# jasperzhong/GNNFlow

Measured on AMD Instinct MI355X. Metric: sampled_edges_per_s, higher is better.
Workload: dtype int64/f32

## Files before the change

### gnnflow_amd/csrc/cache_lru.hip

```cpp
#include "cache_lru_dev.hpp"

#include <algorithm>

namespace gf {

namespace {


__global__ __launch_bounds__(kWide, 8) void lru_list_scan_kernel(Round r, uint32_t row_blocks,
                                                              uint32_t list_blocks,
                                                              uint32_t victim_blocks) {
  const Ctx& c = r.c[blockIdx.y];
  if (!c.update || c.policy != GF_CACHE_LRU || c.fused) return;
  const int tid = threadIdx.x;
  __shared__ uint32_t ws[kWide / 64];
  const uint32_t parity = c.qstate->parity;
  const uint32_t* list = c.queue[parity & 1u];
  constexpr uint32_t kItems = kRowTile / kWide;
  if (blockIdx.x < row_blocks) {
    __shared__ uint32_t carry;
    const uint32_t row_tiles = (c.n + kLruRows - 1) / kLruRows;
    constexpr uint32_t kItems = kLruRows / kWide;
    const uint32_t t_begin = blockIdx.x * c.tiles_per_wg;
    if (t_begin >= row_tiles) return;
    const uint32_t t_end = min(t_begin + c.tiles_per_wg, row_tiles);
    if (tid == 0) carry = 0;
    __syncthreads();
    for (uint32_t t = t_begin; t < t_end; ++t) {
      const uint32_t i0 = t * kLruRows + tid * kItems;
      int32_t sr[kItems];
      int64_t idv[kItems];
#pragma unroll
      for (uint32_t k = 0; k < kItems; ++k) {
        const bool ok = i0 + k < c.n;
        sr[k] = ok ? c.slot_of_row[i0 + k] : -2;
        idv[k] = ok ? c.ids[i0 + k] : 0;
      }
      if (t == t_begin && total_miss(c.ctr) == 0) return;
      uint32_t fm[kItems], lm = 0;
#pragma unroll
      for (uint32_t k = 0; k < kItems; ++k) {
        fm[k] = (sr[k] == -1 && c.map[idv[k]] == -static_cast<int32_t>(i0 + k + 1)) ? 1u : 0u;
        lm += fm[k];
      }
      uint32_t tm;
      uint32_t run = carry + wide_excl_scan(lm, ws, &tm);
#pragma unroll
      for (uint32_t k = 0; k < kItems; ++k) {
        if (i0 + k < c.n && (fm[k] || !c.qmode)) c.rep_flag[i0 + k] = fm[k] ? (kRepMiss | run) : 0u;
        run += fm[k];
      }
      __syncthreads();
      if (tid == 0) carry += tm;
      __syncthreads();
    }
    if (tid == 0) c.row_tile_sum[blockIdx.x] = carry;
    return;
  }
  const uint32_t cap = c.capacity;
  if (blockIdx.x < row_blocks + list_blocks) {
    if (c.qmode) {
      const uint32_t head = c.qstate->head, tail = c.qstate->tail;
      const uint32_t w_lo = head >> 5, w_hi = (tail + 31u) >> 5;
      const uint32_t t0 = w_lo / kBitTile;
      const uint32_t btiles = (w_hi + kBitTile - 1) / kBitTile - t0;
      const bool none = total_miss(c.ctr) == 0;
      for (uint32_t t = blockIdx.x - row_blocks; t < btiles; t += list_blocks) {
        const size_t wi = static_cast<size_t>(t0 + t) * kBitTile + tid * 4;
        const uint4 wd = *reinterpret_cast<const uint4*>(c.qbits + wi);
        if (none) {
          if (wd.x | wd.y | wd.z | wd.w) *reinterpret_cast<uint4*>(c.qbits + wi) = make_uint4(0u, 0u, 0u, 0u);
          continue;
        }
        const uint32_t p0 = __popc(wd.x), p1 = __popc(wd.y), p2 = __popc(wd.z), p3 = __popc(wd.w);
        uint32_t total;
        const uint32_t b = wide_excl_scan(p0 + p1 + p2 + p3, ws, &total);
        uint4* sn = reinterpret_cast<uint4*>(c.wsnap + wi);
        if (wd.x | wd.y) sn[0] = make_uint4(wd.x, b, wd.y, b + p0);
        if (wd.z | wd.w) sn[1] = make_uint4(wd.z, b + p0 + p1, wd.w, b + p0 + p1 + p2);
        if (tid == 0) c.tile_tie[t] = total;
      }
      return;
    }
    const uint32_t list_tiles = (cap + kRowTile - 1) / kRowTile;
    if (blockIdx.x == row_blocks && tid == 0) c.ctr->q_parity = parity;
    bool first = true, staged = false;
    for (uint32_t t = blockIdx.x - row_blocks; t < list_tiles; t += list_blocks) {
      const uint32_t p0 = t * kRowTile + tid * kItems;
      uint32_t sl[kItems], hit[kItems], tc[kItems], local = 0;
#pragma unroll
      for (uint32_t j = 0; j < kItems; ++j) tc[j] = p0 + j < cap ? c.touched[p0 + j] : 0u;
      if (first) {
        uint32_t alt[kItems];
#pragma unroll
        for (uint32_t j = 0; j < kItems; ++j) {
          sl[j] = p0 + j < cap ? c.queue[0][p0 + j] : 0u;
          alt[j] = p0 + j < cap ? c.queue[1][p0 + j] : 0u;
        }
#pragma unroll
        for (uint32_t j = 0; j < kItems; ++j) sl[j] = (parity & 1u) ? alt[j] : sl[j];
        first = false;
        const uint32_t missed = total_miss(c.ctr);
        if (missed == 0) return;
        staged = use_staged_victims(c.stage_tiles, missed, c.stage_min);
      } else {
#pragma unroll
        for (uint32_t j = 0; j < kItems; ++j) sl[j] = p0 + j < cap ? list[p0 + j] : 0u;
      }
#pragma unroll
      for (uint32_t j = 0; j < kItems; ++j) {
        hit[j] = (p0 + j < cap && tc[j] == c.epoch_new) ? 1u : 0u;
        local += hit[j];
      }
      uint32_t total;
      if (staged && t < c.stage_tiles) {
        uint32_t before_hits = wide_excl_scan(local, ws, &total);
        uint32_t at_keep = t * kRowTile + tid * kItems - before_hits;
        uint32_t at_hit = t * kRowTile + before_hits;
#pragma unroll
        for (uint32_t j = 0; j < kItems; ++j) {
          if (p0 + j < cap) {
            if (!hit[j]) c.v_slot[at_keep++] = sl[j];
            else if (c.stage_hits) c.v_pos[at_hit++] = sl[j];
          }
        }
      } else {
        total = wide_sum(local, ws);
      }
      if (tid == 0) {
        c.tile_tie[t] = total;
        if (total) atomicAdd(&c.tile_old[t / kQGroup], total);
      }
    }
    return;
  }
  const uint32_t want = min(total_miss(c.ctr), cap);
  if (c.qmode) {
    const uint32_t vb = blockIdx.x - row_blocks - list_blocks;
    const uint32_t head = c.qstate->head, tail = c.qstate->tail;
    if (vb == 0 && tid == 0) { c.ctr->q_parity = parity; c.ctr->q_head = head; c.ctr->q_tail = tail; }
    if (want == 0) return;
    const uint32_t hbase = head & ~3u, chunks = victim_chunks_used(c, want);
    for (uint32_t ch = vb; ch < chunks; ch += victim_blocks) {
      const uint32_t p0 = hbase + ch * kRowTile + tid * 4;
      uint32_t sl[4];
      const uint32_t mask = victim_walk4(c, list, head, tail, p0, sl);
      uint32_t total;
      uint32_t at = ch * kRowTile + wide_excl_scan(__popc(mask), ws, &total);
#pragma unroll
      for (uint32_t j = 0; j < 4; ++j)
        if (mask & (1u << j)) { c.v_slot[at] = sl[j]; c.v_pos[at] = p0 + j; ++at; }
      if (tid == 0) c.v_count[ch] = total;
    }
    return;
  }
  if (blockIdx.x != row_blocks + list_blocks ||
      use_staged_victims(c.stage_tiles, total_miss(c.ctr), c.stage_min)) return;
  if (want == 0) return;
  uint32_t* kept = c.rep_row;
  uint32_t* moved = c.rep_rank;
  uint32_t found = 0, found_hit = 0;
  for (uint32_t base = 0; base < cap && found < want; base += kRowTile) {
    const uint32_t p0 = base + tid * kItems;
    uint32_t sl[kItems], hit[kItems], lk = 0, lh = 0;
#pragma unroll
    for (uint32_t j = 0; j < kItems; ++j) sl[j] = p0 + j < cap ? list[p0 + j] : 0u;
#pragma unroll
    for (uint32_t j = 0; j < kItems; ++j) {
      const bool in = p0 + j < cap;
      hit[j] = in ? (c.touched[p0 + j] == c.epoch_new ? 1u : 0u) : 2u;
      lk += hit[j] == 0u;
      lh += hit[j] == 1u;
    }
    uint32_t tk, th;
    uint32_t ik = found + wide_excl_scan(lk, ws, &tk);
    uint32_t ih = found_hit + wide_excl_scan(lh, ws, &th);
#pragma unroll
    for (uint32_t j = 0; j < kItems; ++j) {
      if (hit[j] == 0u) { if (ik < want) kept[ik] = sl[j]; ++ik; }
      else if (hit[j] == 1u) { if (ih < want) moved[ih] = sl[j]; ++ih; }
    }
    found += tk;
    found_hit += th;
  }
  if (tid == 0) c.ctr->q_found = min(found, want);
}

__global__ __launch_bounds__(kWide) void lru_list_install_kernel(Round r, uint32_t row_blocks,
                                                                 uint32_t list_blocks) {
  const Ctx& c = r.c[blockIdx.y];
  if (!c.update || c.policy != GF_CACHE_LRU || c.fused || c.qmode) return;
  const int tid = threadIdx.x;
  __shared__ uint32_t ws[kWide / 64];
  const uint32_t row_tiles = (c.n + kLruRows - 1) / kLruRows;
  const uint32_t spans = (row_tiles + c.tiles_per_wg - 1) / c.tiles_per_wg;
  const uint32_t cap = c.capacity;
  if (blockIdx.x < row_blocks) {
    __shared__ uint2 inst[kWide];
    __shared__ int64_t inst_id[kWide];
    __shared__ uint32_t n_inst;
    __shared__ uint32_t s_keep[kMaxStageTiles], s_hitp[kMaxStageTiles], s_nonhit;
    const uint32_t span_rows = c.tiles_per_wg * kLruRows;
    const uint32_t inst_rows = c.inst_rows;
    const uint32_t chunks = (c.n + inst_rows - 1) / inst_rows;
    for (uint32_t chunk = blockIdx.x; chunk < chunks; chunk += row_blocks) {
      const uint32_t i = chunk * inst_rows + tid;
      const bool in = tid < static_cast<int>(inst_rows) && i < c.n;
      const uint32_t code = in ? c.rep_flag[i] : 0u;
      const int64_t id = in ? c.ids[i] : 0;
      const uint32_t w = (chunk * inst_rows) / span_rows;
      uint32_t pm = 0, tm = 0;
      for (uint32_t t = tid; t < spans; t += kWide) {
        const uint32_t m = c.row_tile_sum[t];
        tm += m;
        if (t < w) pm += m;
      }
      const uint32_t q_found = c.ctr->q_found;
      const bool staged = use_staged_victims(c.stage_tiles, total_miss(c.ctr), c.stage_min);
      uint32_t stage_hit = 0, stage_len = 0, th_part = 0;
      if (staged && chunk == blockIdx.x) {
        if (tid < static_cast<int>(c.stage_tiles)) {
          stage_hit = c.tile_tie[tid];
          stage_len = min(kRowTile, cap - tid * kRowTile);
        }
        const uint32_t groups = ((cap + kRowTile - 1) / kRowTile + kQGroup - 1) / kQGroup;
        for (uint32_t g = tid; g < groups; g += kWide) th_part += c.tile_old[g];
      }
      if (chunk == blockIdx.x && total_miss(c.ctr) == 0) return;
      pm = wide_sum(pm, ws);
      tm = wide_sum(tm, ws);
      if (staged && chunk == blockIdx.x) {
        uint32_t unused;
        const uint32_t th = wide_sum(th_part, ws);
        const uint32_t keep_before = wide_excl_scan(stage_len - stage_hit, ws, &unused);
        const uint32_t hit_before = wide_excl_scan(stage_hit, ws, &unused);
        if (tid < static_cast<int>(kMaxStageTiles)) {
          s_keep[tid] = keep_before;
          s_hitp[tid] = hit_before;
        }
        if (tid == 0) s_nonhit = cap - th;
      }
      if (tid == 0) n_inst = 0;
      __syncthreads();
      const uint32_t k = min(tm, cap);
      if (code & kRepMiss) {
        const uint32_t m = pm + (code & kRepRank);
        if (m < k) {
          uint32_t slot;
          int64_t old;
          if (staged) {
            const bool keep = m < s_nonhit;
            const uint32_t x = keep ? m : m - s_nonhit;
            const uint32_t* pref = keep ? s_keep : s_hitp;
            uint32_t lo = 0, hi = c.stage_tiles;
            while (hi - lo > 1) {
              const uint32_t mid = (lo + hi) >> 1;
              if (pref[mid] <= x) lo = mid; else hi = mid;
            }
            const uint32_t at = lo * kRowTile + (x - pref[lo]);
            slot = (keep ? c.v_slot : c.v_pos)[at];
            old = c.slot_id[slot];
          } else {
            slot = m < q_found ? c.rep_row[m] : c.rep_rank[m - q_found];
            old = c.slot_id[slot];
          }
          if (old >= 0) c.map[old] = kAbsent;
          c.slot_id[slot] = id;
          c.map[id] = static_cast<int32_t>(slot);
          const uint32_t at = atomicAdd(&n_inst, 1u);
          inst[at] = make_uint2(slot, i);
          inst_id[at] = id;
        } else {
          c.map[id] = kAbsent;
        }
      }
      __syncthreads();
      const uint32_t total = n_inst * c.dimv;
      if (c.vec4) {
        if (c.inst_rows > kInstRows) copy_installed<float4, 6>(c, inst, inst_id, n_inst, c.dimv * 4, tid);
        else copy_installed<float4, 2>(c, inst, inst_id, n_inst, c.dimv * 4, tid);
      } else if (c.odd4) {
        if (c.inst_rows > kInstRows) copy_installed<uf4, 6>(c, inst, inst_id, n_inst, c.dim, tid);
        else copy_installed<uf4, 2>(c, inst, inst_id, n_inst, c.dim, tid);
      } else {
        for (uint32_t f = tid; c.cache_buf && f < total; f += kWide) {
          const uint32_t j = f / c.dimv, cc = f - j * c.dimv;
          const uint2 pr = inst[j];
          c.cache_buf[static_cast<uint64_t>(pr.x) * c.dimv + cc] =
              c.inst_from_table ? c.feats[static_cast<uint64_t>(inst_id[j]) * c.dimv + cc]
                                : c.out[static_cast<uint64_t>(pr.y) * c.dimv + cc];
        }
      }
      __syncthreads();
    }
    return;
  }
  if (blockIdx.x >= row_blocks + list_blocks) return;
  const uint32_t parity = c.ctr->q_parity;
  const uint32_t* list = c.queue[parity & 1u];
  uint32_t* next = c.queue[(parity & 1u) ^ 1u];
  constexpr uint32_t kSubs = kRowTile / kWide;
  const uint32_t list_tiles = (cap + kRowTile - 1) / kRowTile;
  const uint32_t sub_tiles = (cap + kWide - 1) / kWide;
  const uint32_t groups = (list_tiles + kQGroup - 1) / kQGroup;
  const uint32_t st_first = blockIdx.x - row_blocks;
  uint32_t sl0, tc0;
  {
    const uint32_t p = st_first * kWide + tid;
    const uint32_t a0 = p < cap ? c.queue[0][p] : 0u;
    const uint32_t a1 = p < cap ? c.queue[1][p] : 0u;
    tc0 = p < cap ? c.touched[p] : 0u;
    sl0 = (parity & 1u) ? a1 : a0;
  }
  uint32_t tm = 0, th = 0;
  for (uint32_t t = tid; t < spans; t += kWide) tm += c.row_tile_sum[t];
  for (uint32_t g = tid; g < groups; g += kWide) th += c.tile_old[g];
  if (total_miss(c.ctr) == 0) return;
  tm = wide_sum(tm, ws);
  th = wide_sum(th, ws);
  const uint32_t k = min(tm, cap), n_kept = cap - th;
  for (uint32_t st = st_first; st < sub_tiles; st += list_blocks) {
    const uint32_t t = st / kSubs, q = st - t * kSubs;
    const uint32_t p = st * kWide + tid;
    uint32_t sl, tc;
    if (st == st_first) {
      sl = sl0; tc = tc0;
    } else {
      sl = p < cap ? list[p] : 0u;
      tc = p < cap ? c.touched[p] : 0u;
    }
    uint32_t before = 0;
    const uint32_t g0 = t / kQGroup;
    for (uint32_t g = tid; g < g0; g += kWide) before += c.tile_old[g];
    for (uint32_t u = g0 * kQGroup + tid; u < t; u += kWide) before += c.tile_tie[u];
    for (uint32_t j = 0; j < q; ++j) {
      const uint32_t pj = t * kRowTile + j * kWide + tid;
      before += (pj < cap && c.touched[pj] == c.epoch_new) ? 1u : 0u;
    }
    const uint32_t hit = (p < cap && tc == c.epoch_new) ? 1u : 0u;
    before = wide_sum(before, ws);
    uint32_t total;
    const uint32_t hb = before + wide_excl_scan(hit, ws, &total);
    if (p < cap) {
      const uint32_t l = hit ? n_kept + hb : p - hb;
      const uint32_t at = l < k ? cap - k + l : l - k;
      next[at] = sl;
      c.qpos[sl] = at;
    }
  }
  if (blockIdx.x == row_blocks && tid == 0) c.qstate->parity = parity ^ 1u;
}

__global__ void list_fill_kernel(uint32_t* list, uint32_t first, uint32_t prefix,
                                 const uint32_t* old, uint32_t old_n) {
  const uint32_t stride = gridDim.x * blockDim.x;
  for (uint32_t j = blockIdx.x * blockDim.x + threadIdx.x; j < prefix + old_n; j += stride)
    list[j] = j < prefix ? first + j : old[j - prefix];
}
void lru_list_fill(uint32_t* list, uint32_t first, uint32_t prefix, const uint32_t* old,
                   uint32_t old_n, hipStream_t stream) {
  list_fill_kernel<<<dim3(1024), dim3(256), 0, stream>>>(list, first, prefix, old, old_n);
  GF_HIP(hipGetLastError());
}

struct RoundFork {
  hipStream_t side = nullptr;
  hipEvent_t begin = nullptr, end = nullptr;
  int device = -1;
  ~RoundFork() {
    if (side) (void)hipStreamDestroy(side);
    if (begin) (void)hipEventDestroy(begin);
    if (end) (void)hipEventDestroy(end);
  }
};
inline RoundFork& round_fork() {
  static thread_local RoundFork f;
  return f;
}
inline bool fork_round(hipStream_t stream, hipStream_t* side) {
  RoundFork& f = round_fork();
  int dev = 0;
  GF_HIP(hipGetDevice(&dev));
  if (f.side && f.device != dev) return false;
  if (!f.side) {
    GF_HIP(hipStreamCreateWithFlags(&f.side, hipStreamNonBlocking));
    GF_HIP(hipEventCreateWithFlags(&f.begin, hipEventDisableTiming));
    GF_HIP(hipEventCreateWithFlags(&f.end, hipEventDisableTiming));
    f.device = dev;
  }
  GF_HIP(hipEventRecord(f.begin, stream));
  GF_HIP(hipStreamWaitEvent(f.side, f.begin, 0));
  *side = f.side;
  return true;
}
inline void fork_done() { GF_HIP(hipEventRecord(round_fork().end, round_fork().side)); }
inline void join_round(hipStream_t stream) { GF_HIP(hipStreamWaitEvent(stream, round_fork().end, 0)); }

struct LruExtents {
  size_t fused_list_tiles = 0;
  size_t fused_row_wgs = 0;
  size_t scan_rows = 0;
  size_t scan_row_wgs = 0;
  size_t list_capacity = 0;
  size_t list_inst_wgs = 0;
  size_t queue_bit_tiles = 0;
  size_t queue_victim_wgs = 1;
  size_t queue_rows = 0;
};

LruExtents lru_extents(const Round& r) {
  LruExtents x;
  for (int i = 0; i < r.count; ++i) {
    const Ctx& c = r.c[i];
    if (!c.update || c.policy != GF_CACHE_LRU) continue;
    if (c.fused) {
      x.fused_list_tiles = std::max<size_t>(x.fused_list_tiles, (c.capacity + kFuseTile - 1) / kFuseTile);
      x.fused_row_wgs = std::max<size_t>(x.fused_row_wgs, (c.n + c.fuse_rows - 1) / c.fuse_rows);
      continue;
    }
    const size_t row_tiles = (c.n + kLruRows - 1) / kLruRows;
    x.scan_rows = std::max<size_t>(x.scan_rows, c.n);
    x.scan_row_wgs = std::max(x.scan_row_wgs, (row_tiles + c.tiles_per_wg - 1) / c.tiles_per_wg);
    if (c.qmode) {
      x.queue_bit_tiles = std::max(x.queue_bit_tiles, lru_bit_tiles(c.capacity));
      x.queue_victim_wgs = std::max<size_t>(x.queue_victim_wgs, std::min<size_t>(c.v_chunks, 1024));
      x.queue_rows = std::max<size_t>(x.queue_rows, c.n);
    } else {
      x.list_capacity = std::max<size_t>(x.list_capacity, c.capacity);
      x.list_inst_wgs = std::max<size_t>(x.list_inst_wgs, (c.n + c.inst_rows - 1) / c.inst_rows);
    }
  }
  return x;
}

void launch_list_scan(const Round& r, const LruExtents& x, hipStream_t stream) {
  const unsigned rb = static_cast<unsigned>(x.scan_row_wgs);
  const unsigned lb = static_cast<unsigned>(std::min<size_t>(
      std::max((x.list_capacity + kRowTile - 1) / kRowTile, x.queue_bit_tiles), 1024));
  const unsigned vb = static_cast<unsigned>(x.queue_victim_wgs);
  lru_list_scan_kernel<<<dim3(rb + lb + vb, r.count), dim3(kWide), 0, stream>>>(r, rb, lb, vb);
}

void launch_list_install(const Round& r, const LruExtents& x, hipStream_t stream) {
  const unsigned ib = static_cast<unsigned>(std::min<size_t>(x.list_inst_wgs, 4096));
  const unsigned lb = std::max<unsigned>(
      1, static_cast<unsigned>(std::min<size_t>((x.list_capacity + kWide - 1) / kWide, 1024)));
  lru_list_install_kernel<<<dim3(ib + lb, r.count), dim3(kWide), 0, stream>>>(r, ib, lb);
}

}

void launch_lru_update(const Round& r, hipStream_t stream, bool own_events) {
  const LruExtents x = lru_extents(r);
  hipStream_t side = nullptr;
  const bool forked = x.fused_list_tiles && x.scan_rows && fork_round(stream, &side);
  if (x.fused_list_tiles) {
    launch_lru_fused(r, x.fused_list_tiles, x.fused_row_wgs, forked ? side : stream, own_events);
    if (forked) fork_done();
  }
  if (x.scan_rows) {
    launch_list_scan(r, x, stream);
    if (x.queue_bit_tiles) launch_lru_queue_update(r, x.queue_rows, stream);
    if (x.list_inst_wgs) launch_list_install(r, x, stream);
    GF_HIP(hipGetLastError());
    if (forked) join_round(stream);
  }
}

void FeatureCache::alloc_queue(size_t capacity, hipStream_t stream, DeviceBuffer* old_lists) {
  const bool queue_form = capacity >= queue_min_capacity();
  const size_t queue_cap = lru_queue_cap(capacity, queue_form);
  GF_REQUIRE(!queue_form || queue_cap < (size_t{1} << 30),
             "LRU queue form: more than 2^30 queue positions");
  queue_form_ = queue_form;
  queue_cap_ = queue_cap;
  if (old_lists) {
    old_lists[0] = std::move(queue_);
    old_lists[1] = std::move(queue_alt_);
  }
  auto place = [&](DeviceBuffer& buf, size_t bytes) {
    if (!old_lists) {
      buf.reserve(bytes, 0, stream);
    } else {
      DeviceBuffer fresh;
      fresh.reserve(bytes);
      std::swap(buf, fresh);
    }
  };
  const size_t list_bytes = (queue_cap_ + 16) * sizeof(uint32_t);
  place(queue_, list_bytes);
  place(queue_alt_, list_bytes);
  place(qpos_, std::max<size_t>(capacity, 4) * sizeof(uint32_t));
  if (queue_form_) {
    place(wsnap_, 2 * qbits_bytes(queue_cap_));
    place(qbits_, qbits_bytes(queue_cap_));
    GF_HIP(hipMemsetAsync(qbits_.data(), 0, qbits_bytes(queue_cap_), stream));
    place(compact_, compact_layout(queue_cap_).bytes);
  } else if (!old_lists) {
    wsnap_.release();
    qbits_.release();
    compact_.release();
  }
}

void FeatureCache::init_queue(hipStream_t stream) {
  if (policy_ != GF_CACHE_LRU) return;
  alloc_queue(capacity_, stream, nullptr);
  if (capacity_) lru_list_fill(queue_.as<uint32_t>(), 0u, static_cast<uint32_t>(capacity_), nullptr, 0u, stream);
  const QueueState qs{0u, 0u, 0u, static_cast<uint32_t>(capacity_), 0u, 0u};
  GF_HIP(hipMemcpyAsync(qstate_.data(), &qs, sizeof(qs), hipMemcpyHostToDevice, stream));
  GF_HIP(hipStreamSynchronize(stream));
  tail_bound_ = capacity_;
  index_queue(stream);
}

void FeatureCache::grow_queue(size_t old_capacity, hipStream_t stream) {
  QueueState qs;
  GF_HIP(hipMemcpyAsync(&qs, qstate_.data(), sizeof(qs), hipMemcpyDeviceToHost, stream));
  GF_HIP(hipStreamSynchronize(stream));
  DeviceBuffer old_lists[2];
  alloc_queue(capacity_, stream, old_lists);
  lru_list_fill(queue_.as<uint32_t>(), static_cast<uint32_t>(old_capacity),
                static_cast<uint32_t>(capacity_ - old_capacity), old_lists[qs.parity & 1u].as<uint32_t>(),
                static_cast<uint32_t>(old_capacity), stream);
  const QueueState fresh{0u, 0u, 0u, static_cast<uint32_t>(capacity_), 0u, 0u};
  GF_HIP(hipMemcpyAsync(qstate_.data(), &fresh, sizeof(fresh), hipMemcpyHostToDevice, stream));
  GF_HIP(hipStreamSynchronize(stream));
  tail_bound_ = capacity_;
  index_queue(stream);
  GF_HIP(hipStreamSynchronize(stream));
}

void FeatureCache::index_queue(hipStream_t stream) {
  if (!capacity_) return;
  launch_lru_queue_index(queue_.as<uint32_t>(), queue_alt_.as<uint32_t>(), qstate_.as<QueueState>(),
                         qpos_.as<uint32_t>(), static_cast<uint32_t>(capacity_), stream);
}

void FeatureCache::compact_queue(hipStream_t stream) {
  if (!queue_form_ || tail_bound_ == capacity_) return;
  launch_lru_queue_compact(queue_.as<uint32_t>(), queue_alt_.as<uint32_t>(),
                           qstate_.as<QueueState>(), qpos_.as<uint32_t>(), compact_.as<char>(),
                           compact_layout(queue_cap_), tail_bound_,
                           static_cast<uint32_t>(capacity_), stream);
  tail_bound_ = capacity_;
  ++compactions_;
}

namespace {
inline bool lru_fused_enabled() {
  const char* e = std::getenv("GNNFLOW_LRU_FUSED");
  return e ? std::atoi(e) != 0 : true;
}
}

void FeatureCache::fill_lru_ctx(Ctx& c, size_t n, char* qscratch, hipStream_t stream) {
  const size_t row_tiles = (n + kLruRows - 1) / kLruRows;
  c.tiles_per_wg = static_cast<uint32_t>((row_tiles + kMaxRowTiles - 1) / kMaxRowTiles);
  c.inst_rows = n >= 65536 ? kWide : kInstRows;
  c.queue[0] = queue_.as<uint32_t>();
  c.queue[1] = queue_alt_.as<uint32_t>();
  c.qstate = qstate_.as<QueueState>();
  {
    const size_t stage = align_up(stage_entries(ws_rows_, capacity_) * 4, 256);
    c.v_slot = reinterpret_cast<uint32_t*>(qscratch);
    c.v_pos = reinterpret_cast<uint32_t*>(qscratch + stage);
    c.v_count = reinterpret_cast<uint32_t*>(qscratch + 2 * stage);
    const size_t vc = align_up((victim_chunks(ws_rows_) + 2) * 4, 256) + 256;
    const size_t fst = align_up(fuse_stage_entries(ws_rows_, capacity_) * 8, 256);
    c.v_old = reinterpret_cast<long long*>(qscratch + 2 * stage + vc);
    c.v_hold = reinterpret_cast<long long*>(qscratch + 2 * stage + vc + fst);
    const size_t list_tiles = (capacity_ + kRowTile - 1) / kRowTile;
    const size_t st = std::min(list_tiles, (2 * n + kRowTile - 1) / kRowTile + 2);
    c.stage_tiles = st <= kMaxStageTiles ? static_cast<uint32_t>(st) : 0u;
    c.stage_min = kStageMinWant;
    c.stage_hits = st == list_tiles ? 1 : 0;
  }
  c.qpos = qpos_.as<uint32_t>();
  if (queue_form_) {
    if (n <= capacity_ / 4 && victim_chunks(n) + 1 <= kMaxVChunks) {
      if (tail_bound_ + n > queue_cap_) compact_queue(stream);
      tail_bound_ += n;
      c.qmode = 1;
      c.qbits = qbits_.as<uint32_t>();
      c.wsnap = wsnap_.as<uint2>();
      c.q_group = static_cast<uint32_t>((lru_bit_tiles(capacity_) + kMaxBitGroups - 1) / kMaxBitGroups);
      static const uint32_t forced_group = [] {
        const char* e = std::getenv("GNNFLOW_LRU_QUEUE_GROUP");
        return e ? static_cast<uint32_t>(std::atoi(e)) : 0u;
      }();
      c.q_group = std::max(c.q_group, forced_group);
      c.v_chunks = static_cast<uint32_t>(victim_chunks(n));
      c.stage_tiles = 0;
    } else {
      compact_queue(stream);
      ++list_form_updates_;
    }
  }
  c.fuse_rows = (n > size_t{kInstRows} * kFuseMaxRowWgs || !mirror_) ? kWide : kInstRows;
  if (!c.qmode && lru_fused_enabled() &&
      (capacity_ + kFuseTile - 1) / kFuseTile <= kFuseMaxTiles &&
      (n + c.fuse_rows - 1) / c.fuse_rows <= kFuseMaxRowWgs) {
    if (!granules_.data()) {
      granules_.reserve((kFuseMaxTiles + kFuseMaxRowWgs) * sizeof(unsigned long long), 0, stream);
      GF_HIP(hipMemsetAsync(granules_.data(), 0, granules_.bytes(), stream));
    }
    if (fuse_tag_ == 0xFFFFFFFFu) {
      GF_HIP(hipMemsetAsync(granules_.data(), 0, granules_.bytes(), stream));
      fuse_tag_ = 0;
    }
    c.fused = 1;
    c.trace = trace_.data() ? trace_.as<unsigned long long>() : nullptr;
    c.fuse_tag = ++fuse_tag_;
    c.g_cnt = granules_.as<unsigned long long>();
    c.g_row = c.g_cnt + kFuseMaxTiles;
  }
}

}
```

### gnnflow_amd/csrc/cache_lru_fused.hip

```cpp
#include "cache_lru_dev.hpp"

#include <hip/hip_ext.h>

#include <algorithm>
#include <mutex>
#include <vector>

namespace gf {

namespace {

constexpr uint32_t kFuseSpinsDefault = 1u << 12;
__device__ uint32_t g_fuse_spins = kFuseSpinsDefault;
constexpr int32_t kRepMark = -3;
__device__ unsigned int g_lru_recounts;

#define GF_RLX_AGENT __ATOMIC_RELAXED, __HIP_MEMORY_SCOPE_AGENT

__device__ inline void fuse_poll3(const unsigned long long* g0, const unsigned long long* g1,
                                  const unsigned long long* g2, uint32_t tag, uint32_t* out) {
  const unsigned long long* g[3] = {g0, g1, g2};
  bool need[3], any = false;
#pragma unroll
  for (int k = 0; k < 3; ++k) {
    need[k] = g[k] != nullptr;
    out[k] = need[k] ? ~0u : 0u;
    any |= need[k];
  }
  const uint32_t budget = g_fuse_spins;
  for (uint32_t spins = 0; any && spins < budget; ++spins) {
    unsigned long long x[3];
#pragma unroll
    for (int k = 0; k < 3; ++k) x[k] = need[k] ? __hip_atomic_load(g[k], GF_RLX_AGENT) : 0ull;
    any = false;
#pragma unroll
    for (int k = 0; k < 3; ++k) {
      if (need[k]) {
        if (static_cast<uint32_t>(x[k] >> 32) == tag) {
          out[k] = static_cast<uint32_t>(x[k]);
          need[k] = false;
        } else {
          any = true;
        }
      }
    }
    if (any) __builtin_amdgcn_s_sleep(1);
  }
#pragma unroll
  for (int k = 0; k < 3; ++k)
    if (need[k]) atomicAdd(&g_lru_recounts, 1u);
}

__device__ inline void fuse_publish(unsigned long long* g, uint32_t tag, uint32_t value) {
  __hip_atomic_store(g, (static_cast<unsigned long long>(tag) << 32) | value, GF_RLX_AGENT);
}

__device__ inline uint32_t total_hits(const Counters* c) {
  uint32_t h = 0;
#pragma unroll
  for (int i = 0; i < kShards; ++i) h += c->shard[i].hits;
  return h;
}

__device__ inline uint32_t fuse_parity(const Ctx& c) {
  const unsigned long long w = *reinterpret_cast<const unsigned long long*>(c.qstate);
  const uint32_t parity = static_cast<uint32_t>(w), flip = static_cast<uint32_t>(w >> 32);
  return (flip == c.fuse_tag ? parity ^ 1u : parity) & 1u;
}

__device__ inline uint32_t fuse_recount_tile(const Ctx& c, uint32_t t) {
  uint32_t h = 0;
  const uint32_t lo = t * kFuseTile, hi = min(lo + kFuseTile, c.capacity);
  for (uint32_t p = lo; p < hi; ++p) h += c.touched[p] == c.epoch_new ? 1u : 0u;
  return h;
}

__device__ inline uint32_t fuse_recount_rows(const Ctx& c, uint32_t b) {
  uint32_t m = 0;
  const uint32_t lo = b * c.fuse_rows, hi = min(lo + c.fuse_rows, c.n);
  for (uint32_t i = lo; i < hi; ++i) {
    const int64_t id = c.ids[i];
    if (id < 0 || static_cast<uint64_t>(id) >= c.num_ids) continue;
    const int32_t claim = __hip_atomic_load(&c.map[id], GF_RLX_AGENT);
    const int32_t sr = __hip_atomic_load(&c.slot_of_row[i], GF_RLX_AGENT);
    if (sr == kRepMark || (sr == -1 && claim == -static_cast<int32_t>(i + 1))) ++m;
  }
  return m;
}

__device__ inline uint32_t fuse_walk_tile(const Ctx& c, const uint32_t* list, uint32_t t,
                                          uint32_t x, bool want_hit) {
  const uint32_t lo = t * kFuseTile, hi = min(lo + kFuseTile, c.capacity);
  uint32_t seen = 0;
  for (uint32_t p = lo; p < hi; ++p) {
    const bool hit = c.touched[p] == c.epoch_new;
    if (hit == want_hit) {
      if (seen == x) return list[p];
      ++seen;
    }
  }
  return list[lo];
}

#define GF_STAMP(k) \
  do { if (c.trace && threadIdx.x == 0) c.trace[4 + vx * 8 + (k)] = wall_clock64(); } while (0)

__global__ __launch_bounds__(kWide) void lru_list_fused_kernel(Round r, uint32_t count_blocks,
                                                               uint32_t row_blocks,
                                                               uint32_t write_blocks) {
  const Ctx& c = r.c[blockIdx.y];
  asm volatile("" :: "s"(c.update), "s"(c.policy), "s"(c.fused), "s"(c.trace), "s"(c.n),
               "s"(c.capacity), "s"(c.fuse_tag), "s"(c.fuse_rows), "s"(c.touched), "s"(c.queue[0]),
               "s"(c.queue[1]), "s"(c.qstate), "s"(c.ctr), "s"(c.epoch_new), "s"(c.slot_id),
               "s"(c.ids), "s"(c.map), "s"(c.slot_of_row), "s"(c.g_cnt), "s"(c.g_row),
               "s"(c.v_slot), "s"(c.v_old), "s"(c.v_pos), "s"(c.v_hold), "s"(c.qpos),
               "s"(c.num_ids), "s"(c.cache_buf));
  const uint32_t vx = blockIdx.x;
  if (!c.update || c.policy != GF_CACHE_LRU || !c.fused) return;
  const int tid = threadIdx.x;
  if (c.trace && vx == 0 && tid == 0) {
    c.trace[0] = count_blocks; c.trace[1] = row_blocks; c.trace[2] = write_blocks; c.trace[3] = c.fuse_tag;
  }
  GF_STAMP(0);
  __shared__ uint32_t ws[kWide / 64];
  const uint32_t cap = c.capacity, tag = c.fuse_tag;
  const uint32_t tiles = (cap + kFuseTile - 1) / kFuseTile;
  const uint32_t row_wgs = (c.n + c.fuse_rows - 1) / c.fuse_rows;

  if (vx < count_blocks) {
    bool first = true;
    uint32_t par = 0, bound = 0;
    bool stage_hits = false;
    for (uint32_t t = vx; t < tiles; t += count_blocks) {
      const uint32_t p = t * kFuseTile + tid;
      const bool in = p < cap;
      const uint32_t tc = in ? c.touched[p] : 0u;
      uint32_t sl;
      if (first) {
        const uint32_t a0 = in ? c.queue[0][p] : 0u;
        const uint32_t a1 = in ? c.queue[1][p] : 0u;
        par = fuse_parity(c);
        const uint32_t missed = total_miss(c.ctr);
        if (missed == 0) return;
        const uint32_t hit_rows = total_hits(c.ctr);
        const uint32_t want = min(missed, cap);
        bound = min(cap, want + hit_rows);
        stage_hits = static_cast<uint64_t>(want) + hit_rows > cap;
        sl = par ? a1 : a0;
        first = false;
      } else {
        sl = in ? c.queue[par][p] : 0u;
      }
      const bool hit = in && tc == c.epoch_new;
      const bool stage = t * kFuseTile < bound;
      if (t == vx) GF_STAMP(1);
      long long old = -1;
      if (stage && in && (!hit || stage_hits)) old = c.slot_id[sl];
      uint32_t total;
      const uint32_t hb = wide_excl_scan(hit ? 1u : 0u, ws, &total);
      if (stage && in) {
        if (!hit) {
          const uint32_t at = t * kFuseTile + (tid - hb);
          __hip_atomic_store(&c.v_slot[at], sl, GF_RLX_AGENT);
          __hip_atomic_store(&c.v_old[at], old, GF_RLX_AGENT);
        } else if (stage_hits) {
          const uint32_t at = t * kFuseTile + hb;
          __hip_atomic_store(&c.v_pos[at], sl, GF_RLX_AGENT);
          __hip_atomic_store(&c.v_hold[at], old, GF_RLX_AGENT);
        }
      }
      asm volatile("s_waitcnt vmcnt(0)" ::: "memory");
      __syncthreads();
      if (tid == 0) fuse_publish(&c.g_cnt[t], tag, total);
      if (t == vx) GF_STAMP(2);
    }
    return;
  }

  __shared__ uint32_t s_keep[kFuseMaxTiles + 1], s_hitp[kFuseMaxTiles + 1];
  __shared__ uint32_t s_direct;

  if (vx < count_blocks + row_blocks) {
    const uint32_t b = vx - count_blocks;
    if (b >= row_wgs) return;
    __shared__ uint2 inst[kWide];
    __shared__ int64_t inst_id[kWide];
    __shared__ uint32_t n_inst;
    const uint32_t i = b * c.fuse_rows + tid;
    const bool in = tid < static_cast<int>(c.fuse_rows) && i < c.n;
    const int32_t sr = in ? c.slot_of_row[i] : -2;
    const int64_t id = in ? c.ids[i] : 0;
    const uint32_t par = fuse_parity(c);
    if (total_miss(c.ctr) == 0) return;
    const bool fm = sr == -1 && c.map[id] == -static_cast<int32_t>(i + 1);
    if (fm) {
      __hip_atomic_store(&c.slot_of_row[i], kRepMark, GF_RLX_AGENT);
      asm volatile("s_waitcnt vmcnt(0)" ::: "memory");
    }
    uint32_t cnt;
    const uint32_t rank = wide_excl_scan(fm ? 1u : 0u, ws, &cnt);
    if (tid == 0) {
      fuse_publish(&c.g_row[b], tag, cnt);
      n_inst = 0;
      s_direct = 0;
    }
    GF_STAMP(1);
    constexpr uint32_t kPer = kFuseMaxTiles / kWide;
    static_assert(kPer == 2 && kFuseMaxRowWgs <= kWide, "fuse_poll3: one row + two count granules");
    uint32_t pv[3];
    fuse_poll3(static_cast<uint32_t>(tid) < b ? &c.g_row[tid] : nullptr,
               tid * kPer < tiles ? &c.g_cnt[tid * kPer] : nullptr,
               tid * kPer + 1 < tiles ? &c.g_cnt[tid * kPer + 1] : nullptr, tag, pv);
    if (pv[0] == ~0u) pv[0] = fuse_recount_rows(c, tid);
    GF_STAMP(5);
    const uint32_t pm = wide_sum(pv[0], ws);
    GF_STAMP(6);
    uint32_t hv[kPer], run_h = 0;
#pragma unroll
    for (uint32_t k = 0; k < kPer; ++k) {
      hv[k] = pv[1 + k];
      if (hv[k] == ~0u) {
        hv[k] = fuse_recount_tile(c, tid * kPer + k);
        s_direct = 1u;
      }
      run_h += hv[k];
    }
    uint32_t th;
    uint32_t hb = wide_excl_scan(run_h, ws, &th);
#pragma unroll
    for (uint32_t k = 0; k < kPer; ++k) {
      const uint32_t t = tid * kPer + k;
      if (t <= tiles) {
        s_hitp[t] = hb;
        s_keep[t] = min(t * kFuseTile, cap) - hb;
      }
      hb += hv[k];
    }
    __syncthreads();
    GF_STAMP(2);
    const uint32_t n_kept = cap - th;
    if (fm) {
      const uint32_t m = pm + rank;
      if (m < cap) {
        const bool keep = m < n_kept;
        const uint32_t x = keep ? m : m - n_kept;
        const uint32_t* pref = keep ? s_keep : s_hitp;
        uint32_t lo = 0, hi = tiles;
        while (hi - lo > 1) {
          const uint32_t mid = (lo + hi) >> 1;
          if (pref[mid] <= x) lo = mid; else hi = mid;
        }
        uint32_t slot;
        long long old;
        if (s_direct) {
          slot = fuse_walk_tile(c, c.queue[par], lo, x - pref[lo], !keep);
          old = c.slot_id[slot];
        } else {
          const uint32_t at = lo * kFuseTile + (x - pref[lo]);
          slot = __hip_atomic_load(keep ? &c.v_slot[at] : &c.v_pos[at], GF_RLX_AGENT);
          old = __hip_atomic_load(keep ? &c.v_old[at] : &c.v_hold[at], GF_RLX_AGENT);
        }
        if (old >= 0) c.map[old] = kAbsent;
        c.slot_id[slot] = id;
        c.map[id] = static_cast<int32_t>(slot);
        const uint32_t at = atomicAdd(&n_inst, 1u);
        inst[at] = make_uint2(slot, i);
        inst_id[at] = id;
      } else {
        c.map[id] = kAbsent;
      }
    }
    __syncthreads();
    GF_STAMP(3);
    const uint32_t total = n_inst * c.dimv;
    if (c.vec4) {
      if (c.fuse_rows > kInstRows) copy_installed<float4, 6>(c, inst, inst_id, n_inst, c.dimv * 4, tid);
      else copy_installed<float4, 2>(c, inst, inst_id, n_inst, c.dimv * 4, tid);
    } else if (c.odd4) {
      if (c.fuse_rows > kInstRows) copy_installed<uf4, 6>(c, inst, inst_id, n_inst, c.dim, tid);
      else copy_installed<uf4, 2>(c, inst, inst_id, n_inst, c.dim, tid);
    } else {
      for (uint32_t f = tid; c.cache_buf && f < total; f += kWide) {
        const uint32_t j = f / c.dimv, cc = f - j * c.dimv;
        const uint2 pr = inst[j];
        c.cache_buf[static_cast<uint64_t>(pr.x) * c.dimv + cc] =
            c.inst_from_table ? c.feats[static_cast<uint64_t>(inst_id[j]) * c.dimv + cc]
                              : c.out[static_cast<uint64_t>(pr.y) * c.dimv + cc];
      }
    }
    GF_STAMP(4);
    return;
  }

  const uint32_t wb = vx - count_blocks - row_blocks;
  if (wb >= write_blocks || wb >= tiles) return;
  uint32_t sl0, tc0, par;
  {
    const uint32_t p = wb * kFuseTile + tid;
    const uint32_t a0 = p < cap ? c.queue[0][p] : 0u;
    const uint32_t a1 = p < cap ? c.queue[1][p] : 0u;
    tc0 = p < cap ? c.touched[p] : 0u;
    par = fuse_parity(c);
    sl0 = par ? a1 : a0;
  }
  if (total_miss(c.ctr) == 0) return;
  __builtin_amdgcn_s_sleep(32);
  __builtin_amdgcn_s_sleep(32);
  constexpr uint32_t kPer = kFuseMaxTiles / kWide;
  uint32_t pv[3];
  fuse_poll3(static_cast<uint32_t>(tid) < row_wgs ? &c.g_row[tid] : nullptr,
             tid * kPer < tiles ? &c.g_cnt[tid * kPer] : nullptr,
             tid * kPer + 1 < tiles ? &c.g_cnt[tid * kPer + 1] : nullptr, tag, pv);
  if (pv[0] == ~0u) pv[0] = fuse_recount_rows(c, tid);
  const uint32_t tm = wide_sum(pv[0], ws);
  uint32_t hv[kPer], run_h = 0;
#pragma unroll
  for (uint32_t k = 0; k < kPer; ++k) {
    hv[k] = pv[1 + k];
    if (hv[k] == ~0u) hv[k] = fuse_recount_tile(c, tid * kPer + k);
    run_h += hv[k];
  }
  uint32_t th;
  uint32_t hbt = wide_excl_scan(run_h, ws, &th);
#pragma unroll
  for (uint32_t k = 0; k < kPer; ++k) {
    const uint32_t t = tid * kPer + k;
    if (t <= tiles) s_hitp[t] = hbt;
    hbt += hv[k];
  }
  __syncthreads();
  GF_STAMP(1);
  const uint32_t k = min(tm, cap), n_kept = cap - th;
  const uint32_t* list = c.queue[par];
  uint32_t* next = c.queue[par ^ 1u];
  for (uint32_t t = wb; t < tiles; t += write_blocks) {
    const uint32_t p = t * kFuseTile + tid;
    uint32_t sl, tc;
    if (t == wb) {
      sl = sl0; tc = tc0;
    } else {
      sl = p < cap ? list[p] : 0u;
      tc = p < cap ? c.touched[p] : 0u;
    }
    const uint32_t hit = (p < cap && tc == c.epoch_new) ? 1u : 0u;
    uint32_t total;
    const uint32_t hb = s_hitp[t] + wide_excl_scan(hit, ws, &total);
    if (p < cap) {
      const uint32_t l = hit ? n_kept + hb : p - hb;
      const uint32_t at = l < k ? cap - k + l : l - k;
      next[at] = sl;
      c.qpos[sl] = at;
    }
  }
  GF_STAMP(2);
  if (wb == 0 && tid == 0) {
    *reinterpret_cast<unsigned long long*>(c.qstate) =
        (static_cast<unsigned long long>(tag) << 32) | (par ^ 1u);
  }
}

__device__ __attribute__((used)) uint32_t wide_sum_unfolded(uint32_t v, uint32_t* ws) {
  return wide_sum(v, ws);
}

}

void launch_lru_fused(const Round& r, size_t list_tiles, size_t row_wgs, hipStream_t stream,
                      bool own_events) {
  const unsigned cb = static_cast<unsigned>(std::min<size_t>(list_tiles, 1024));
  const unsigned rb = static_cast<unsigned>(std::max<size_t>(row_wgs, 1));
  const unsigned wb = static_cast<unsigned>(std::min<size_t>(list_tiles, kFuseMaxTiles));
  hipEvent_t e0 = nullptr, e1 = nullptr;
  if (own_events && profile_begin(kProfLru, &e0, &e1)) {
    hipExtLaunchKernelGGL(lru_list_fused_kernel, dim3(cb + rb + wb, r.count), dim3(kWide), 0, stream,
                          e0, e1, 0, r, cb, rb, wb);
    profile_end(kProfLru, e0, e1);
  } else {
    lru_list_fused_kernel<<<dim3(cb + rb + wb, r.count), dim3(kWide), 0, stream>>>(r, cb, rb, wb);
  }
  GF_HIP(hipGetLastError());
}

void lru_fuse_spins_from_env(int device) {
  static std::mutex mu;
  static std::vector<int> done;
  std::lock_guard<std::mutex> lk(mu);
  if (std::find(done.begin(), done.end(), device) == done.end()) {
    done.push_back(device);
    if (const char* v = std::getenv("GNNFLOW_LRU_FUSE_SPINS")) {
      const uint32_t spins = static_cast<uint32_t>(std::atoll(v));
      GF_HIP(hipMemcpyToSymbol(HIP_SYMBOL(g_fuse_spins), &spins, sizeof(spins)));
    }
  }
}

uint64_t lru_recounts() {
  unsigned int v = 0;
  GF_HIP(hipMemcpyFromSymbol(&v, HIP_SYMBOL(g_lru_recounts), sizeof(v)));
  return v;
}

}
```

### gnnflow_amd/csrc/feature_cache_ctx.hpp

```cpp
#pragma once

#include "feature_cache.hpp"
#include "owner_hash.hpp"

#include <cstdlib>
#include <cstring>

namespace gf {

constexpr int32_t kAbsent = INT32_MIN;
constexpr int kThreads = 256;
constexpr int kWide = 1024;
constexpr int kFine = 2048;
constexpr int kBins1 = 4096;
constexpr int kBins2 = 2048;
constexpr uint32_t kAgeMax = kFine + 2048u * 2048u - 1u;
constexpr int kTile = 1024;
constexpr int kRing = 32;
constexpr int kMaxCtx = 4;
constexpr uint32_t kRowTile = 4096;
constexpr uint32_t kMaxRowTiles = 1024;
constexpr uint32_t kQGroup = 64;
constexpr uint32_t kInstRows = 256;
constexpr uint32_t kLruRows = 1024;
constexpr uint32_t kMaxStageTiles = 1024;
constexpr uint32_t kBitTile = 4096;
constexpr uint32_t kMaxBitGroups = 1024;
constexpr uint32_t kMaxVChunks = 2048;
constexpr uint32_t kFuseTile = kWide;
constexpr uint32_t kFuseMaxTiles = 2048;
constexpr uint32_t kFuseMaxRowWgs = 1024;

constexpr int kShards = 8;
struct Shard {
  uint32_t hits;
  uint32_t n_miss;
  uint32_t pad[30];
};
struct Counters {
  Shard shard[kShards];
  uint32_t n_unique;
  uint32_t th_age;
  uint32_t th_k_tie;
  uint32_t fifo_start;
  uint32_t ticket;
  uint32_t q_parity;
  uint32_t q_found;
  uint32_t q_head;
  uint32_t q_tail;
  uint32_t pad[23];
};
constexpr uint32_t kCounterWords = sizeof(Counters) / 4;

struct QueueState { uint32_t parity, flip_tag, head, tail, lone_walks, pad; };

struct Ctx {
  const int64_t* ids;
  uint32_t n;
  int vec4;
  uint32_t dimv;
  int odd4;
  uint32_t dim, tail;
  int inst_from_table;
  uint32_t tile_rows;
  uint32_t pad0;
  float* out;
  const float* feats;
  const float* miss_rows;
  const uint32_t* miss_index;
  const uint32_t* req_pos;
  const int32_t* remap;
  uint32_t* flag;
  const unsigned long long* pmap;
  const float* ring;
  uint32_t st_lo, st_span, st_mask, st_cap;
  uint32_t* progress;
  uint32_t progress_val;
  unsigned long long* st_fallback;
  unsigned long long* trace;
  uint64_t num_ids;
  int32_t* map;
  float* cache_buf;
  int64_t* slot_id;
  uint32_t* stamp;
  uint32_t* touched;
  uint32_t* queue[2];
  QueueState* qstate;
  uint32_t tiles_per_wg;
  uint32_t inst_rows;
  int qmode;
  uint32_t* qpos;
  uint32_t* qbits;
  uint2* wsnap;
  uint32_t q_group;
  uint32_t stage_tiles;
  uint32_t stage_min;
  int stage_hits;
  uint32_t v_chunks;
  uint32_t* v_slot;
  uint32_t* v_pos;
  uint32_t* v_count;
  int fused;
  uint32_t fuse_tag;
  uint32_t fuse_rows;
  unsigned long long* g_cnt;
  unsigned long long* g_row;
  long long* v_old;
  long long* v_hold;
  uint32_t capacity;
  uint32_t epoch_new;
  int update;
  int policy;
  uint32_t* fifo_ptr;
  int32_t* slot_of_row;
  uint32_t* rep_flag;
  uint32_t* rep_rank;
  uint32_t* rep_row;
  int64_t* rep_id;
  uint32_t* row_tile_sum;
  uint32_t* hist1;
  uint32_t* hist2;
  uint32_t* tile_tie;
  uint32_t* tile_old;
  Counters* ctr;
  Counters* ctr_next;
  uint32_t* stats;
};
struct Round {
  Ctx c[kMaxCtx];
  int count;
};

__device__ inline uint32_t total_miss(const Counters* c) {
  uint32_t m = 0;
#pragma unroll
  for (int i = 0; i < kShards; ++i) m += c->shard[i].n_miss;
  return m;
}

constexpr uint32_t kStageMinWant = 8192;

typedef float uf4 __attribute__((ext_vector_type(4), aligned(4)));

typedef float nf4 __attribute__((ext_vector_type(4)));
__device__ inline void nt_store(float v, float* p) { __builtin_nontemporal_store(v, p); }
__device__ inline void nt_store(const float4& v, float4* p) {
  nf4 t; t.x = v.x; t.y = v.y; t.z = v.z; t.w = v.w;
  __builtin_nontemporal_store(t, reinterpret_cast<nf4*>(p));
}

template <typename VecT> __device__ inline VecT global_load(const void* p);
template <> __device__ inline float global_load<float>(const void* p) {
  return *(const __attribute__((address_space(1))) float*)p;
}
template <> __device__ inline uf4 global_load<uf4>(const void* p) {
  return *(const __attribute__((address_space(1))) uf4*)p;
}
template <> __device__ inline float4 global_load<float4>(const void* p) {
  const nf4 t = *(const __attribute__((address_space(1))) nf4*)p;
  return make_float4(t.x, t.y, t.z, t.w);
}

template <typename VecT> __device__ inline VecT vec_zero();
template <> __device__ inline uf4 vec_zero<uf4>() { return uf4{0.f, 0.f, 0.f, 0.f}; }
__device__ inline void nt_store(const uf4& v, uf4* p) { __builtin_nontemporal_store(v, p); }
template <> __device__ inline float vec_zero<float>() { return 0.0f; }
template <> __device__ inline float4 vec_zero<float4>() { return make_float4(0.f, 0.f, 0.f, 0.f); }

constexpr uint32_t kRepMiss = 1u << 31, kRepRank = kRepMiss - 1u;
constexpr uint32_t kRepHit = 1u << 30, kRepPos = kRepHit - 1u;

constexpr uint32_t kGatherTraceBase = 4u + 8u * (2u * 2048u + 1024u);
constexpr uint32_t kGatherTraceWgs = 1024u;

struct StageCtx {
  const int64_t* ids;
  uint32_t n;
  const int32_t* map;
  uint64_t num_ids;
  unsigned long long* pmap;
  uint32_t* region_rows;
  long long* region_ids;
  uint32_t gen, lo, mask, cap;
  const uint32_t* qpos;
  const QueueState* qstate;
  uint32_t risk;
};
struct StageRound {
  StageCtx c[kMaxCtx];
  int count;
};

struct PullJob {
  const long long* ids;
  const float* feats;
  float* dst;
  uint32_t* region_rows;
  uint32_t* next_rows;
  unsigned long long* pulled;
  uint32_t cap, dim, vec4;
};
struct PullJobs {
  PullJob j[2];
  int count;
};

struct PullCtx {
  const int64_t* ids;
  uint32_t n;
  const int64_t* key_base;
  const int64_t* key_index;
  int32_t* map;
  uint64_t num_ids;
  uint32_t* counts;
  uint32_t cstride;
  uint32_t* cursor;
  int64_t* send_ids;
  uint32_t* req_pos;
};
struct PullRound {
  PullCtx c[kMaxCtx];
  int count;
  OwnerDiv od;
};

inline void set_odd4(Ctx& c, size_t dim, bool allowed) {
  c.dim = static_cast<uint32_t>(dim);
  c.odd4 = 0;
  c.tail = 0;
  if (c.vec4 || !allowed || dim < 8) return;
  c.odd4 = 1;
  c.dimv = static_cast<uint32_t>((dim + 3) / 4);
  c.tail = static_cast<uint32_t>(dim % 4);
}

inline bool vec4_ok(size_t dim, const void* a, const void* b, const void* c) {
  auto al = [](const void* p) { return (reinterpret_cast<uintptr_t>(p) & 15u) == 0; };
  return dim % 4 == 0 && al(a) && al(b) && al(c);
}

inline size_t queue_min_capacity() {
  const char* v = std::getenv("GNNFLOW_LRU_QUEUE_MIN_CAPACITY");
  return v ? static_cast<size_t>(std::atoll(v)) : (size_t{1} << 19);
}

inline size_t lru_queue_cap(size_t capacity, bool queue_form) {
  return queue_form ? capacity + capacity / 2 + 64 : capacity;
}

inline size_t qbits_bytes(size_t queue_cap) {
  const size_t words = (queue_cap + 64 + 31) / 32;
  return ((words + kRowTile - 1) / kRowTile + 1) * kRowTile * sizeof(uint32_t);
}

inline size_t lru_bit_tiles(size_t capacity) {
  return ((lru_queue_cap(capacity, true) + 64) / 32 + kBitTile - 1) / kBitTile + 1;
}

struct CompactLayout { size_t live_bits, tile_cnt, group_sum, state, bytes; };
inline CompactLayout compact_layout(size_t queue_cap) {
  const size_t tiles = (queue_cap + kRowTile - 1) / kRowTile + 1;
  const size_t groups = (tiles + kQGroup - 1) / kQGroup + 1;
  CompactLayout l;
  l.live_bits = 0;
  l.tile_cnt = l.live_bits + align_up(tiles * (kRowTile / 64) * 8, 256);
  l.group_sum = l.tile_cnt + align_up(tiles * 4, 256);
  l.state = l.group_sum + align_up(groups * 4, 256);
  l.bytes = l.state + 256;
  return l;
}

inline size_t victim_chunks(size_t n) { return (2 * n + kRowTile - 1) / kRowTile + 2; }

inline size_t stage_entries(size_t n, size_t capacity) {
  const size_t list_tiles = (capacity + kRowTile - 1) / kRowTile;
  const size_t list_form = std::min<size_t>(std::min(list_tiles, victim_chunks(n)), kMaxStageTiles);
  return std::max(list_form, victim_chunks(n)) * kRowTile + n;
}

inline size_t fuse_stage_entries(size_t n, size_t capacity) {
  return (std::min(n, capacity) / kFuseTile + 2) * kFuseTile;
}

inline uint32_t pick_tile_rows(size_t n) {
  uint32_t t = 64;
  while (t > 16 && (n + t - 1) / t < 1024) t >>= 1;
  return t;
}

Ctx plain_ctx(const float* feats, size_t num_rows, size_t dim, const int64_t* ids, size_t n,
              float* out);
void launch_gather(Round& r, hipStream_t stream);
void launch_lru_update(const Round& r, hipStream_t stream, bool own_events);
void lru_fuse_spins_from_env(int device);
void launch_select_update(const Round& r, hipStream_t stream);
void launch_round(Round& r, hipStream_t stream);

}
```

Before: 755.6 million.

## Pad fused-LRU granules to 128-byte lines and poll only needed count tiles

Each per-tile and per-row-workgroup granule word used for cross-workgroup signalling in the fused LRU kernel now sits on its own 128-byte stride instead of being packed 8 bytes apart. This is meant to stop atomic publishes and polls on neighbouring granules from contending on the same cache line. When all victims fit in the front of the list, row workgroups also bound their polling and binary search to the tiles covering the victim range, so they skip waiting on later count tiles. The cost is a 16x larger granule buffer and an extra branch that relies on the front-victim condition being correct.

```diff
diff --git a/gnnflow_amd/csrc/cache_lru.hip b/gnnflow_amd/csrc/cache_lru.hip
--- a/gnnflow_amd/csrc/cache_lru.hip
+++ b/gnnflow_amd/csrc/cache_lru.hip
@@ -602,7 +602,7 @@
       (capacity_ + kFuseTile - 1) / kFuseTile <= kFuseMaxTiles &&
       (n + c.fuse_rows - 1) / c.fuse_rows <= kFuseMaxRowWgs) {
     if (!granules_.data()) {
-      granules_.reserve((kFuseMaxTiles + kFuseMaxRowWgs) * sizeof(unsigned long long), 0, stream);
+      granules_.reserve(granule_bytes(), 0, stream);
       GF_HIP(hipMemsetAsync(granules_.data(), 0, granules_.bytes(), stream));
     }
     if (fuse_tag_ == 0xFFFFFFFFu) {
@@ -613,8 +613,8 @@
     c.trace = trace_.data() ? trace_.as<unsigned long long>() : nullptr;
     c.fuse_tag = ++fuse_tag_;
     c.g_cnt = granules_.as<unsigned long long>();
-    c.g_row = c.g_cnt + kFuseMaxTiles;
-  }
-}
-
-}
+    c.g_row = granule_at(c.g_cnt, kFuseMaxTiles);
+  }
+}
+
+}
diff --git a/gnnflow_amd/csrc/cache_lru_fused.hip b/gnnflow_amd/csrc/cache_lru_fused.hip
--- a/gnnflow_amd/csrc/cache_lru_fused.hip
+++ b/gnnflow_amd/csrc/cache_lru_fused.hip
@@ -60,6 +60,12 @@
 #pragma unroll
   for (int i = 0; i < kShards; ++i) h += c->shard[i].hits;
   return h;
+}
+
+__device__ inline bool fuse_victims_in_front(const Ctx& c, uint32_t missed, uint32_t* bound) {
+  const uint32_t hit_rows = total_hits(c.ctr), want = min(missed, c.capacity);
+  *bound = min(c.capacity, want + hit_rows);
+  return static_cast<uint64_t>(want) + hit_rows <= c.capacity;
 }
 
 __device__ inline uint32_t fuse_parity(const Ctx& c) {
@@ -142,10 +148,7 @@
         par = fuse_parity(c);
         const uint32_t missed = total_miss(c.ctr);
         if (missed == 0) return;
-        const uint32_t hit_rows = total_hits(c.ctr);
-        const uint32_t want = min(missed, cap);
-        bound = min(cap, want + hit_rows);
-        stage_hits = static_cast<uint64_t>(want) + hit_rows > cap;
+        stage_hits = !fuse_victims_in_front(c, missed, &bound);
         sl = par ? a1 : a0;
         first = false;
       } else {
@@ -171,7 +174,7 @@
       }
       asm volatile("s_waitcnt vmcnt(0)" ::: "memory");
       __syncthreads();
-      if (tid == 0) fuse_publish(&c.g_cnt[t], tag, total);
+      if (tid == 0) fuse_publish(granule_at(c.g_cnt, t), tag, total);
       if (t == vx) GF_STAMP(2);
     }
     return;
@@ -191,7 +194,8 @@
     const int32_t sr = in ? c.slot_of_row[i] : -2;
     const int64_t id = in ? c.ids[i] : 0;
     const uint32_t par = fuse_parity(c);
-    if (total_miss(c.ctr) == 0) return;
+    const uint32_t missed = total_miss(c.ctr);
+    if (missed == 0) return;
     const bool fm = sr == -1 && c.map[id] == -static_cast<int32_t>(i + 1);
     if (fm) {
       __hip_atomic_store(&c.slot_of_row[i], kRepMark, GF_RLX_AGENT);
@@ -200,17 +204,20 @@
     uint32_t cnt;
     const uint32_t rank = wide_excl_scan(fm ? 1u : 0u, ws, &cnt);
     if (tid == 0) {
-      fuse_publish(&c.g_row[b], tag, cnt);
+      fuse_publish(granule_at(c.g_row, b), tag, cnt);
       n_inst = 0;
       s_direct = 0;
     }
     GF_STAMP(1);
+    uint32_t bound;
+    const bool front = fuse_victims_in_front(c, missed, &bound);
+    const uint32_t look = front ? (bound + kFuseTile - 1) / kFuseTile : tiles;
     constexpr uint32_t kPer = kFuseMaxTiles / kWide;
     static_assert(kPer == 2 && kFuseMaxRowWgs <= kWide, "fuse_poll3: one row + two count granules");
     uint32_t pv[3];
-    fuse_poll3(static_cast<uint32_t>(tid) < b ? &c.g_row[tid] : nullptr,
-               tid * kPer < tiles ? &c.g_cnt[tid * kPer] : nullptr,
-               tid * kPer + 1 < tiles ? &c.g_cnt[tid * kPer + 1] : nullptr, tag, pv);
+    fuse_poll3(static_cast<uint32_t>(tid) < b ? granule_at(c.g_row, tid) : nullptr,
+               tid * kPer < look ? granule_at(c.g_cnt, tid * kPer) : nullptr,
+               tid * kPer + 1 < look ? granule_at(c.g_cnt, tid * kPer + 1) : nullptr, tag, pv);
     if (pv[0] == ~0u) pv[0] = fuse_recount_rows(c, tid);
     GF_STAMP(5);
     const uint32_t pm = wide_sum(pv[0], ws);
@@ -242,10 +249,10 @@
     if (fm) {
       const uint32_t m = pm + rank;
       if (m < cap) {
-        const bool keep = m < n_kept;
+        const bool keep = front || m < n_kept;
         const uint32_t x = keep ? m : m - n_kept;
         const uint32_t* pref = keep ? s_keep : s_hitp;
-        uint32_t lo = 0, hi = tiles;
+        uint32_t lo = 0, hi = look;
         while (hi - lo > 1) {
           const uint32_t mid = (lo + hi) >> 1;
           if (pref[mid] <= x) lo = mid; else hi = mid;
@@ -308,9 +315,9 @@
   __builtin_amdgcn_s_sleep(32);
   constexpr uint32_t kPer = kFuseMaxTiles / kWide;
   uint32_t pv[3];
-  fuse_poll3(static_cast<uint32_t>(tid) < row_wgs ? &c.g_row[tid] : nullptr,
-             tid * kPer < tiles ? &c.g_cnt[tid * kPer] : nullptr,
-             tid * kPer + 1 < tiles ? &c.g_cnt[tid * kPer + 1] : nullptr, tag, pv);
+  fuse_poll3(static_cast<uint32_t>(tid) < row_wgs ? granule_at(c.g_row, tid) : nullptr,
+             tid * kPer < tiles ? granule_at(c.g_cnt, tid * kPer) : nullptr,
+             tid * kPer + 1 < tiles ? granule_at(c.g_cnt, tid * kPer + 1) : nullptr, tag, pv);
   if (pv[0] == ~0u) pv[0] = fuse_recount_rows(c, tid);
   const uint32_t tm = wide_sum(pv[0], ws);
   uint32_t hv[kPer], run_h = 0;
diff --git a/gnnflow_amd/csrc/feature_cache_ctx.hpp b/gnnflow_amd/csrc/feature_cache_ctx.hpp
--- a/gnnflow_amd/csrc/feature_cache_ctx.hpp
+++ b/gnnflow_amd/csrc/feature_cache_ctx.hpp
@@ -30,6 +30,9 @@
 constexpr uint32_t kFuseTile = kWide;
 constexpr uint32_t kFuseMaxTiles = 2048;
 constexpr uint32_t kFuseMaxRowWgs = 1024;
+constexpr uint32_t kGranuleStride = 128;
+static_assert(kGranuleStride >= 8 && (kGranuleStride & (kGranuleStride - 1)) == 0,
+              "granules are naturally aligned 8-byte words");
 
 constexpr int kShards = 8;
 struct Shard {
@@ -282,6 +285,13 @@
   return (std::min(n, capacity) / kFuseTile + 2) * kFuseTile;
 }
 
+__host__ __device__ inline unsigned long long* granule_at(unsigned long long* base, uint32_t i) {
+  return base + static_cast<size_t>(i) * (kGranuleStride / sizeof(unsigned long long));
+}
+inline size_t granule_bytes() {
+  return static_cast<size_t>(kFuseMaxTiles + kFuseMaxRowWgs) * kGranuleStride;
+}
+
 inline uint32_t pick_tile_rows(size_t n) {
   uint32_t t = 64;
   while (t > 16 && (n + t - 1) / t < 1024) t >>= 1;
```

Result: slower. 726.8 million (-3.8%).
